# flo-audio/flo

Hardware: AMD Instinct MI355X
Metric: Msamples/s encoded (44.1k stereo, q=high) (higher is better)
Workload: dtype f32

## Files before the change

### flo_amd/csrc/lossy_device.hpp

```cpp
#pragma once
#include <hip/hip_runtime.h>
#include <stdint.h>

#include "pack_rows.h"

namespace flo {


struct LossyDevTables {
    const float4 *pack;
    const float4 *pack_g;
    const float4 *pack_ext;
    const float *ath_db;
    const uint8_t *band;
    const float *band_count;
    const float *s10d;
    const uint32_t *lane_bnd;
    const uint32_t *lane_slot0;
    const uint32_t *band_slot0;
    int max_band_slots;
    uint32_t dirty;
    float smr_thr;
    int q_transparent;
};
// ... 418 lines not shown
    v2f c2r = a4r - a6r, c2i = a4i - a6i;
    v2f c1r = a5r + a7i, c1i = a5i - a7r;
    v2f c3r = a5r - a7i, c3i = a5i + a7r;
    const v2f e1r = c1r + c1i, e1i = c1i - c1r;
    const v2f e3r = c3i - c3r, e3i = c3r + c3i;
    xr[0] = b0r + c0r; xi[0] = b0i + c0i;
    xr[4] = b0r - c0r; xi[4] = b0i - c0i;
    xr[1] = fma2(e1r, s, b1r); xi[1] = fma2(e1i, s, b1i);
    xr[5] = fma2(-e1r, s, b1r); xi[5] = fma2(-e1i, s, b1i);
    xr[2] = b2r + c2i; xi[2] = b2i - c2r;
    xr[6] = b2r - c2i; xi[6] = b2i + c2r;
    xr[3] = fma2(e3r, s, b3r); xi[3] = fma2(-e3i, s, b3i);
    xr[7] = fma2(-e3r, s, b3r); xi[7] = fma2(e3i, s, b3i);
}

__device__ __forceinline__ void cmul_2(v2f &xr, v2f &xi, float wr, float wi) {
    const v2f WR = splat2(wr), WI = splat2(wi);
    v2f r = fma2(xr, WR, -(xi * WI));
    v2f i = fma2(xr, WI, xi * WR);
    xr = r;
    xi = i;
}
__device__ __forceinline__ void cmul_2_pair(v2f &xr, v2f &xi, v2f w) {
    const v2f WR = splat2(w.x);
    v2f r = fma2(xr, WR, -mul2_hi(xi, w));
    v2f i = fma2_a_hi_c(xr, w, xi * WR);
    xr = r;
    xi = i;
}

struct NoShadow { __device__ __forceinline__ void operator()() const {} };
template <typename F = NoShadow>
__device__ __forceinline__ void fft512_2(const int lane, v2f (&zr)[8], v2f (&zi)[8], float4 *x4, const LossyDevTables &T, F &&shadow = F()) {
    dft8_2(zr, zi);
#pragma unroll
    for (int kk = 0; kk < 4; kk++) {
        const float4 w = T.pack[(kRowF1 + kk) * 64 + lane];
        cmul_2(zr[2 * kk + 1], zi[2 * kk + 1], w.x, w.y);
        if (kk < 3) cmul_2_pair(zr[2 * kk + 2], zi[2 * kk + 2], (v2f){w.z, w.w});
    }
    {
        const int nb = lane >> 3, nc = lane & 7;
#pragma unroll
        for (int ka = 0; ka < 8; ka++) x4[(8 * ka + nc) * kXchStride + nb] = make_float4(zr[ka].x, zr[ka].y, zi[ka].x, zi[ka].y);
        wave_sync();
#pragma unroll
        for (int r = 0; r < 8; r++) {
            const float4 v = x4[lane * kXchStride + r];
            zr[r] = (v2f){v.x, v.y};
            zi[r] = (v2f){v.z, v.w};
        }
        shadow();
        wave_sync();
    }
    dft8_2(zr, zi);
#pragma unroll
    for (int kk = 0; kk < 4; kk++) {
        const float4 w = T.pack[(kRowF2 + kk) * 64 + lane];
        cmul_2(zr[2 * kk + 1], zi[2 * kk + 1], w.x, w.y);
        if (kk < 3) cmul_2_pair(zr[2 * kk + 2], zi[2 * kk + 2], (v2f){w.z, w.w});
    }
    {
        const int ka = lane >> 3, nc = lane & 7;
#pragma unroll
        for (int kb = 0; kb < 8; kb++) x4[(ka + 8 * kb) * kXchStride + nc] = make_float4(zr[kb].x, zr[kb].y, zi[kb].x, zi[kb].y);
        wave_sync();
#pragma unroll
        for (int r = 0; r < 8; r++) {
            const float4 v = x4[lane * kXchStride + r];
            zr[r] = (v2f){v.x, v.y};
            zi[r] = (v2f){v.z, v.w};
        }
        wave_sync();
    }
    dft8_2(zr, zi);
}

__device__ __forceinline__ void cmul_2_tw(v2f &xr, v2f &xi, v2f w) {
    const v2f r = fma2_a_lo_nc(xr, w, mul2_hi(xi, w));
    const v2f i = fma2_a_hi_c(xr, w, mul2_lo(xi, w));
    xr = r;
    xi = i;
}
template <typename F = NoShadow>
__device__ __forceinline__ void fft512_2_tw(const int lane, v2f (&zr)[8], v2f (&zi)[8], float4 *x4, const v4f (&f1)[4],
                                            const v4f (&f2)[4], F &&shadow = F()) {
    dft8_2(zr, zi);
#pragma unroll
    for (int kk = 0; kk < 4; kk++) {
        cmul_2_tw(zr[2 * kk + 1], zi[2 * kk + 1], f1[kk].xy);
        if (kk < 3) cmul_2_tw(zr[2 * kk + 2], zi[2 * kk + 2], f1[kk].zw);
    }
    {
        const int nb = lane >> 3, nc = lane & 7;
#pragma unroll
        for (int ka = 0; ka < 8; ka++) x4[(8 * ka + nc) * kXchStride + nb] = make_float4(zr[ka].x, zr[ka].y, zi[ka].x, zi[ka].y);
        wave_sync();
#pragma unroll
        for (int r = 0; r < 8; r++) {
            const float4 v = x4[lane * kXchStride + r];
            zr[r] = (v2f){v.x, v.y};
            zi[r] = (v2f){v.z, v.w};
        }
        shadow();
        wave_sync();
    }
    dft8_2(zr, zi);
#pragma unroll
    for (int kk = 0; kk < 4; kk++) {
        cmul_2_tw(zr[2 * kk + 1], zi[2 * kk + 1], f2[kk].xy);
        if (kk < 3) cmul_2_tw(zr[2 * kk + 2], zi[2 * kk + 2], f2[kk].zw);
    }
    {
        const int ka = lane >> 3, nc = lane & 7;
#pragma unroll
        for (int kb = 0; kb < 8; kb++) x4[(ka + 8 * kb) * kXchStride + nc] = make_float4(zr[kb].x, zr[kb].y, zi[kb].x, zi[kb].y);
        wave_sync();
#pragma unroll
        for (int r = 0; r < 8; r++) {
            const float4 v = x4[lane * kXchStride + r];
            zr[r] = (v2f){v.x, v.y};
            zi[r] = (v2f){v.z, v.w};
        }
        wave_sync();
    }
    dft8_2(zr, zi);
}

__device__ __forceinline__ void load_half_fast_2(const int lane, const float *__restrict__ pcm, long long s0, v2f (&he)[8], v2f (&ho)[8]) {
    const char *base0 = reinterpret_cast<const char *>(pcm + s0 * 2);
    const char *base1 = base0 + 4096;
    const unsigned va = 16u * (unsigned)lane, vb = 16u * (unsigned)(63 - lane);
#pragma unroll
    for (int r = 0; r < 8; r++) {
        const int rr = r & 3;
        const char *pe = (r < 4 ? base1 : base0) + va + 1024 * rr;
        const char *po = (r < 4 ? base0 : base1) + vb + (3080 - 1024 * rr);
        const float2 a = *reinterpret_cast<const float2 *>(pe);
        const float2 b = *reinterpret_cast<const float2 *>(po);
        he[r] = (v2f){a.x, a.y};
        ho[r] = (v2f){b.x, b.y};
    }
}

__device__ __forceinline__ void fold_2(const int lane, const v2f (&ae)[8], const v2f (&ao)[8], const v2f (&be)[8], const v2f (&bo)[8],
                                       v2f (&zr)[8], v2f (&zi)[8], const LossyDevTables &T) {
    float4 t4;
#pragma unroll
    for (int r = 0; r < 8; r++) {
        const float4 ww = T.pack[(kRowWin + r) * 64 + lane];
        const v2f wae = splat2(ww.x), wao = splat2(ww.y), wbe = splat2(ww.z);
        const v2f whi = {ww.z, ww.w};
        if (!(r & 1)) t4 = pack_row(&T.pack[(kRowTw + (r >> 1)) * 64 + lane]);
        const v2f wx = splat2((r & 1) ? t4.z : t4.x);
        const v2f thi = {t4.z, t4.w};
        v2f re, im;
        if (r < 4) {
            re = fma2_na_hi_nc(bo[r], whi, be[r] * wbe);
            im = fma2(ao[r], wao, -(ae[r] * wae));
        } else {
            re = fma2(-ao[r], wao, ae[r] * wae);
            im = fma2_na_hi_nc(bo[r], whi, be[r] * wbe);
        }
        if (r & 1) {
            zr[r] = fma2_na_hi_nc(im, thi, re * wx);
            zi[r] = fma2_a_hi_nc(re, thi, im * wx);
        } else {
            const v2f wy = splat2(t4.y);
            zr[r] = fma2(-im, wy, -(re * wx));
            zi[r] = fma2(re, wy, -(im * wx));
        }
    }
}

__device__ __forceinline__ void post_rotate_transpose_2(const int lane, const v2f (&zr)[8], const v2f (&zi)[8], float2 *c2,
                                                        v2f (&c)[16], const LossyDevTables &T) {
    const int pl = 2 * lane + 2 * (lane >> 3);
    float2 *const w0 = c2 + pl;
    float2 *const w1 = c2 + (1149 - 7 * 144) - pl;
    float4 t4;
#pragma unroll
    for (int r = 0; r < 8; r++) {
        if (!(r & 1)) t4 = pack_row(&T.pack[(kRowTw + (r >> 1)) * 64 + lane]);
        const v2f wx = splat2((r & 1) ? t4.z : t4.x);
        v2f R, I;
        if (r & 1) {
            const v2f thi = {t4.z, t4.w};
            R = fma2_na_hi_nc(zi[r], thi, zr[r] * wx);
            I = fma2(zi[r], wx, -mul2_hi(zr[r], thi));
        } else {
            const v2f wy = splat2(t4.y);
            R = fma2(-zi[r], wy, -(zr[r] * wx));
            I = fma2(zi[r], wx, -(zr[r] * wy));
        }
        w0[144 * r] = make_float2(R.x, R.y);
        w1[144 * (7 - r)] = make_float2(I.x, I.y);
    }
    wave_sync();
    const float4 *p = reinterpret_cast<const float4 *>(&c2[18 * lane]);
#pragma unroll
    for (int q = 0; q < 8; q++) {
        const float4 v = p[q];
        c[2 * q] = (v2f){v.x, v.y};
        c[2 * q + 1] = (v2f){v.z, v.w};
    }
    wave_sync();
}

__device__ __forceinline__ v2f fold_a_part(const int r, const v2f he, const v2f ho, const float4 ww) {
    const v2f wae = splat2(ww.x), wao = splat2(ww.y);
    return r < 4 ? fma2(ho, wao, -(he * wae)) : fma2(-ho, wao, he * wae);
}
__device__ __forceinline__ void fold_carry_init_2(const int lane, v2f (&acar)[8], const LossyDevTables &T) {
#pragma unroll
    for (int r = 0; r < 8; r++) acar[r] = fold_a_part(r, splat2(0.f), splat2(0.f), T.pack[(kRowWin + r) * 64 + lane]);
}
__device__ __forceinline__ void fold_carry_2(const int lane, const v2f (&ne)[8], const v2f (&no)[8], v2f (&acar)[8],
                                             const v4f (&tw)[4], v2f (&zr)[8], v2f (&zi)[8], const LossyDevTables &T) {
#pragma unroll
    for (int r = 0; r < 8; r++) {
        const float4 ww = T.pack[(kRowWin + r) * 64 + lane];
        const v2f wbe = splat2(ww.z);
        const v2f whi = {ww.z, ww.w};
        const v2f t2 = (r & 1) ? tw[r >> 1].zw : tw[r >> 1].xy;
        const v2f bp = fma2_na_hi_nc(no[r], whi, ne[r] * wbe);
        const v2f re = r < 4 ? bp : acar[r], im = r < 4 ? acar[r] : bp;
        zr[r] = fma2_na_hi_nc(im, t2, mul2_lo(re, t2));
        zi[r] = fma2_a_hi_nc(re, t2, mul2_lo(im, t2));
        acar[r] = fold_a_part(r, ne[r], no[r], ww);
    }
}

__device__ __forceinline__ void post_rotate_transpose_2_tw(const int lane, const v2f (&zr)[8], const v2f (&zi)[8], float2 *c2,
                                                           v2f (&c)[16], const v4f (&tw)[4]) {
    const int pl = 2 * lane + 2 * (lane >> 3);
    float2 *const w0 = c2 + pl;
    float2 *const w1 = c2 + (1149 - 7 * 144) - pl;
#pragma unroll
    for (int r = 0; r < 8; r++) {
        const v2f t2 = (r & 1) ? tw[r >> 1].zw : tw[r >> 1].xy;
        const v2f R = fma2_na_hi_nc(zi[r], t2, mul2_lo(zr[r], t2));
        const v2f I = fma2_a_lo_nc(zi[r], t2, mul2_hi(zr[r], t2));
        w0[144 * r] = make_float2(R.x, R.y);
        w1[144 * (7 - r)] = make_float2(I.x, I.y);
    }
    wave_sync();
    const float4 *p = reinterpret_cast<const float4 *>(&c2[18 * lane]);
#pragma unroll
    for (int q = 0; q < 8; q++) {
        const float4 v = p[q];
        c[2 * q] = (v2f){v.x, v.y};
        c[2 * q + 1] = (v2f){v.z, v.w};
    }
    wave_sync();
}

struct LaneConst {
    float rcount;
};

__device__ __forceinline__ void load_lane_const(const int lane, LaneConst &L, const LossyDevTables &T) {
    L.rcount = T.pack[kRowLane * 64 + lane].z;
}

constexpr int kZeroSlot = kSlotCap + 64;

template <int CH>
__device__ __forceinline__ void band_stats(const int lane, const float (&c)[CH][16], float2 (*slots)[kSlotCap + 64 + 1],
                                           const LossyDevTables &T, float (&energy)[CH], float (&bmax)[CH]) {
    float kp[16];
    uint32_t dv[16], so[12];
#pragma unroll
    for (int g = 0; g < 4; g++) {
        const float4 keep = T.pack[(kRowKeep + g) * 64 + lane];
        const float4 dsto = T.pack[(kRowDst + g) * 64 + lane];
        kp[4 * g + 0] = keep.x, kp[4 * g + 1] = keep.y, kp[4 * g + 2] = keep.z, kp[4 * g + 3] = keep.w;
        dv[4 * g + 0] = __float_as_uint(dsto.x), dv[4 * g + 1] = __float_as_uint(dsto.y);
        dv[4 * g + 2] = __float_as_uint(dsto.z), dv[4 * g + 3] = __float_as_uint(dsto.w);
    }
#pragma unroll
    for (int g = 0; g < 3; g++) {
        const float4 lst = T.pack[(kRowLst + g) * 64 + lane];
        so[4 * g + 0] = __float_as_uint(lst.x), so[4 * g + 1] = __float_as_uint(lst.y);
        so[4 * g + 2] = __float_as_uint(lst.z), so[4 * g + 3] = __float_as_uint(lst.w);
    }
    __builtin_amdgcn_sched_barrier(0);
    float acc[CH], mx[CH];
#pragma unroll
    for (int ch = 0; ch < CH; ch++) {
        acc[ch] = 0.f;
        mx[ch] = 0.f;
    }
#pragma unroll
    for (int e = 0; e < 16; e++) {
#pragma unroll
        for (int ch = 0; ch < CH; ch++) {
            acc[ch] = fmaf(c[ch][e], c[ch][e], acc[ch]);
            mx[ch] = max_abs_raw(mx[ch], c[ch][e]);
            *reinterpret_cast<float2 *>(reinterpret_cast<char *>(slots[ch]) + dv[e]) = make_float2(acc[ch], mx[ch]);
            acc[ch] *= kp[e];
            mx[ch] *= kp[e];
        }
    }
    wave_sync();
// ... 164 lines not shown
}

__device__ __forceinline__ float masking_amplitude(float s, float smr_thr) {
    const float thr_db = s - 10.0f;
    return __builtin_amdgcn_exp2f((smr_thr + thr_db) * 0.16609640474436813f);
}

__device__ __forceinline__ uint32_t sf_word(float sf) {
    if (sf > 1e-10f) {
        float v = __builtin_amdgcn_logf(sf) * 256.0f + 32768.0f;
        v = __builtin_amdgcn_fmed3f(v, 0.0f, 65535.0f);
        return (uint32_t)v;
    }
    return 0u;
}

__device__ __forceinline__ float round_away(float x) {
    float t = truncf(x);
    float d = x - t;
    return t + truncf(d + d);
}

template <int CH, bool EXACT>
__device__ __forceinline__ void quantise(const int lane, const float (&c)[CH][16], const WaveLds<CH> &lds, const LaneConst &L,
                                         const LossyDevTables &T, int (&q)[CH][16]) {
    float al[16];
    uint32_t bo[16];
#pragma unroll
    for (int g = 0; g < 4; g++) {
        const float4 al4 = T.pack[(kRowAth + g) * 64 + lane];
        const float4 bo4 = T.pack[(kRowBo + g) * 64 + lane];
        al[4 * g + 0] = al4.x, al[4 * g + 1] = al4.y, al[4 * g + 2] = al4.z, al[4 * g + 3] = al4.w;
        bo[4 * g + 0] = __float_as_uint(bo4.x), bo[4 * g + 1] = __float_as_uint(bo4.y);
        bo[4 * g + 2] = __float_as_uint(bo4.z), bo[4 * g + 3] = __float_as_uint(bo4.w);
    }
    __builtin_amdgcn_sched_barrier(0);
    float2 bv[CH][16];
#pragma unroll
    for (int e = 0; e < 16; e++)
#pragma unroll
        for (int ch = 0; ch < CH; ch++)
            bv[ch][e] = *reinterpret_cast<const float2 *>(reinterpret_cast<const char *>(lds.bandv[ch]) + bo[e]);
    __builtin_amdgcn_sched_barrier(0);
#pragma unroll
    for (int e = 0; e < 16; e++) {
#pragma unroll
        for (int ch = 0; ch < CH; ch++) {
            const float x = c[ch][e];
            const float ax = fabsf(x);
            const float thr = max_raw(bv[ch][e].x, al[e]);
            const float xs = x * bv[ch][e].y;
            const float half = __uint_as_float((__float_as_uint(xs) & 0x80000000u) | 0x3EFFFFFFu);
            const int v = cvt_rz(xs + half);
            if (EXACT) {
                bool keep = ax > thr;
                const bool near = fabsf(ax - thr) <= 1e-5f * thr || (T.q_transparent && !(ax > 1e-10f));
                if (near) {
                    float signal_db = ax > 1e-10f ? 20.0f * log10f(ax) : -100.0f;
                    float sdb = *reinterpret_cast<const float *>(reinterpret_cast<const char *>(lds.band_s[ch]) + (bo[e] >> 1));
                    float t = fmaxf(sdb, T.ath_db[16 * lane + e]) - 10.0f;
                    keep = (signal_db - t) > T.smr_thr;
                }
                q[ch][e] = keep ? v : 0;
            } else {
                const int mask = __float_as_int(thr - ax) >> 31;
                q[ch][e] = v & mask;
            }
        }
    }
}

constexpr int kSlots = kSlotCap + 64 + 1;
struct StereoLds {
    union {
        float4 xch4[kXch4];
        float2 coef2[kCoef2];
        struct {
            float4 slot[kSlots];
            float4 ts[32];
        } a;
    } u;
};

template <uint32_t DIRTY = 0xFFFFu, bool SO_PRE = false, bool MASKS = false>
__device__ __forceinline__ void band_stats_2(const int lane, const v2f (&c)[16], float4 *slot, const LossyDevTables &T,
                                             float &energy1, float &bmax1, const uint32_t *so_pre = nullptr,
                                             const unsigned long long *close = nullptr, const uint32_t slot_first = 0) {
    static_assert(!MASKS || SO_PRE, "the masked form takes its addresses from band_stats_2_prepare");
    typedef float v4f __attribute__((ext_vector_type(4)));
    typedef __attribute__((address_space(3))) v4f lds_v4f;
    const uint32_t s0 = (uint32_t)__builtin_amdgcn_readfirstlane((int)(uint32_t)(uintptr_t)slot);
    if (!SO_PRE) {
        typedef __attribute__((address_space(3))) float lds_f32;
        float z = 0.f;
        asm volatile("" : "+v"(z));
        *reinterpret_cast<lds_f32 *>((uintptr_t)(s0 + 16u * (uint32_t)kZeroSlot + 4u * ((uint32_t)lane & 3u))) = z;
    }
    uint32_t so[12];
#pragma unroll
    for (int g = 0; g < 3; g++) {
        if (SO_PRE) {
            so[4 * g + 0] = so_pre[4 * g + 0], so[4 * g + 1] = so_pre[4 * g + 1], so[4 * g + 2] = so_pre[4 * g + 2], so[4 * g + 3] = so_pre[4 * g + 3];
        } else {
            const float4 lst = T.pack[(kRowLst + g) * 64 + lane];
            so[4 * g + 0] = s0 + 2u * __float_as_uint(lst.x), so[4 * g + 1] = s0 + 2u * __float_as_uint(lst.y);
            so[4 * g + 2] = s0 + 2u * __float_as_uint(lst.z), so[4 * g + 3] = s0 + 2u * __float_as_uint(lst.w);
        }
    }
    const uint32_t dirty = DIRTY;
    v4f am = {0.f, 0.f, 0.f, 0.f};
    uint32_t sa = slot_first;
#pragma unroll
    for (int g = 0; g < 4; g++) {
        const float4 keep = MASKS ? make_float4(0.f, 0.f, 0.f, 0.f) : pack_row(&T.pack[(kRowKeep + g) * 64 + lane]);
        const float4 dsto = MASKS ? make_float4(0.f, 0.f, 0.f, 0.f) : pack_row(&T.pack[(kRowDst + g) * 64 + lane]);
        const float kp[4] = {keep.x, keep.y, keep.z, keep.w};
        const uint32_t dv[4] = {__float_as_uint(dsto.x), __float_as_uint(dsto.y), __float_as_uint(dsto.z), __float_as_uint(dsto.w)};
#pragma unroll
        for (int k = 0; k < 4; k++) {
            const int e = 4 * g + k;
            am.xy = fma2(c[e], c[e], am.xy);
            const bool prev_open = e > 0 && !((dirty >> (e - 1)) & 1u), this_open = e < 15 && !((dirty >> e) & 1u);
            if (prev_open) {
                am.z = max3_abs_raw(am.z, c[e - 1].x, c[e].x);
                am.w = max3_abs_raw(am.w, c[e - 1].y, c[e].y);
            } else if (!this_open) {
                am.z = max_abs_raw(am.z, c[e].x);
                am.w = max_abs_raw(am.w, c[e].y);
            }
            if (MASKS && ((dirty >> e) & 1u)) {
                if (e < 15) {
                    v2f lo = am.xy, hi = am.zw;
                    unsigned long long saved;
                    asm volatile("s_and_saveexec_b64 %[sv], %[m]\n\t"
                                 "ds_write2_b64 %[a], %[lo], %[hi] offset1:1\n\t"
                                 "v_add_u32 %[a], 16, %[a]\n\t"
                                 "v_pk_mul_f32 %[lo], %[lo], 0 op_sel_hi:[1,0]\n\t"
                                 "v_pk_mul_f32 %[hi], %[hi], 0 op_sel_hi:[1,0]\n\t"
                                 "s_mov_b64 exec, %[sv]"
                                 : [a] "+v"(sa), [lo] "+v"(lo), [hi] "+v"(hi), [sv] "=&s"(saved)
                                 : [m] "s"(close[e])
                                 : "memory");
                    am.xy = lo, am.zw = hi;
                } else {
                    *reinterpret_cast<lds_v4f *>((uintptr_t)sa) = am;
                }
            } else if ((dirty >> e) & 1u) {
                *reinterpret_cast<lds_v4f *>((uintptr_t)(s0 + 2u * dv[k])) = am;
                if (e < 15) {
                    am.xy = am.xy * splat2(kp[k]);
                    am.zw = am.zw * splat2(kp[k]);
                }
            }
        }
    }
    wave_sync();
    v2f energy = splat2(0.f), bmax = splat2(0.f);
#pragma unroll
    for (int g = 0; g < 3; g++) {
        v4f v[4];
#pragma unroll
        for (int u = 0; u < 4; u++) v[u] = *reinterpret_cast<const lds_v4f *>((uintptr_t)so[4 * g + u]);
#pragma unroll
        for (int u = 0; u < 4; u++) energy = energy + (v2f){v[u].x, v[u].y};
#pragma unroll
        for (int u = 0; u < 4; u += 2) {
            bmax.x = max3_raw(bmax.x, v[u].z, v[u + 1].z);
            bmax.y = max3_raw(bmax.y, v[u].w, v[u + 1].w);
        }
    }
    const int groups = (T.max_band_slots + 7) >> 3;
    for (int g = 3; g < groups; g++) {
        const float4 lst = g < 6 ? T.pack_g[(kRowLstCold + g - 3) * 64 + lane] : T.pack_ext[(g - 6) * 64 + lane];
        const uint32_t sx[4] = {__float_as_uint(lst.x), __float_as_uint(lst.y), __float_as_uint(lst.z), __float_as_uint(lst.w)};
        v4f w[4];
#pragma unroll
        for (int u = 0; u < 4; u++) w[u] = *reinterpret_cast<const lds_v4f *>((uintptr_t)(s0 + 2u * sx[u]));
#pragma unroll
        for (int u = 0; u < 4; u++) {
            energy = energy + (v2f){w[u].x, w[u].y};
            bmax.x = max_raw(bmax.x, w[u].z);
            bmax.y = max_raw(bmax.y, w[u].w);
        }
    }
    {
        const auto e2 = __builtin_amdgcn_permlane32_swap(__float_as_int(energy.x), __float_as_int(energy.y), false, false);
        const auto m2 = __builtin_amdgcn_permlane32_swap(__float_as_int(bmax.x), __float_as_int(bmax.y), false, false);
        energy1 = __int_as_float(e2[0]) + __int_as_float(e2[1]);
        bmax1 = max_raw(__int_as_float(m2[0]), __int_as_float(m2[1]));
    }
    wave_sync();
}

__device__ __forceinline__ void band_stats_2_prepare(const int lane, float4 *slot, const float4 *pack, uint32_t (&so)[12],
                                                     uint32_t &slot_first) {
    const uint32_t s0 = (uint32_t)(uintptr_t)slot;
    slot_first = s0 + 16u * reinterpret_cast<const uint32_t *>(pack + kRowLane * 64 + lane)[1];
    if (lane < 4) reinterpret_cast<float *>(slot + kZeroSlot)[lane] = 0.f;
#pragma unroll
    for (int g = 0; g < 3; g++) {
        const float4 lst = pack[(kRowLst + g) * 64 + lane];
        so[4 * g + 0] = s0 + 2u * __float_as_uint(lst.x), so[4 * g + 1] = s0 + 2u * __float_as_uint(lst.y);
        so[4 * g + 2] = s0 + 2u * __float_as_uint(lst.z), so[4 * g + 3] = s0 + 2u * __float_as_uint(lst.w);
    }
}
template <uint32_t DIRTY>
__device__ __forceinline__ void band_stats_2_masks(const StatMasks *masks, unsigned long long (&close)[16]) {
#pragma unroll
    for (int e = 0; e < 16; e++) {
        const bool used = e < 15 && ((DIRTY >> e) & 1u);
        close[e] = used ? masks->close[e] : 0ull;
        if (used) asm volatile("" : "+s"(close[e]));
    }
}

struct QuantRows {
    float4 bo4[4];
};
__device__ __forceinline__ void quant_rows_load(const int lane, const LossyDevTables &T, QuantRows &R) {
#pragma unroll
    for (int g = 0; g < 4; g++) {
        R.bo4[g] = T.pack[(kRowBo + g) * 64 + lane];
    }
}
__device__ __forceinline__ void quantise_2(const int lane, const v2f (&c)[16], const float4 *ts, const LossyDevTables &T,
                                           const QuantRows &R, uint32_t (&xs)[2][8]) {
    typedef float v4f __attribute__((ext_vector_type(4)));
    typedef __attribute__((address_space(3))) v4f lds_f4;
    const uint32_t ts0 = (uint32_t)__builtin_amdgcn_readfirstlane((int)(uint32_t)(uintptr_t)ts);
    const uint32_t sgn_mask = 0x7FFFFFFFu;
    uint32_t phalf = 0x3EFFFFFFu;
    asm volatile("" : "+v"(phalf));
#pragma unroll
    for (int g = 0; g < 4; g++) {
        const float4 al4 = T.pack[(kRowAth + g) * 64 + lane];
        const float4 bo4 = R.bo4[g];
        const float al[4] = {al4.x, al4.y, al4.z, al4.w};
        const uint32_t bo[4] = {__float_as_uint(bo4.x), __float_as_uint(bo4.y), __float_as_uint(bo4.z), __float_as_uint(bo4.w)};
        v4f tb[4];
#pragma unroll
        for (int k = 0; k < 4; k++) tb[k] = *reinterpret_cast<const lds_f4 *>((uintptr_t)(ts0 + 2u * bo[k]));
        int v[2][4];
// ... 548 lines not shown
```

### flo_amd/csrc/lossy_kernels.hip

```cpp
#include <assert.h>
#include <stdlib.h>

#include <mutex>
#include <set>
#include <type_traits>
#include <utility>

#include "chain2q_roles.hpp"
#include "crc_device.hpp"
#include "lossy_device.hpp"
#include "lossy_kernels.hpp"
#include "../../include/flo_synth.h"

#ifndef FLO_SKIP
#define FLO_SKIP 0
#endif
#define FLO_KEEP(x) asm volatile("" ::"v"(x))
#ifdef FLO_STAMPS
#define STAMP(i)                                                                                  \
    do {                                                                                          \
        __builtin_amdgcn_sched_barrier(0);                                                        \
        unsigned long long t_;                                                                    \
        asm volatile("s_memtime %0\n\ts_waitcnt lgkmcnt(0)" : "=s"(t_)::"memory");              \
        __builtin_amdgcn_sched_barrier(0);                                                        \
// ... 616 lines not shown
    float ath_floor = masks->band_ath_floor[lane & 31];
    asm volatile("" : "+v"(ath_floor));
    v4f tw[4];
    v4f f1[4], f2[4];
    if (!COEFFS) {
#pragma unroll
        for (int k = 0; k < 4; k++) tw[k] = pack_row_v(&T.pack[(kRowTw + k) * 64 + lane]);
#pragma unroll
        for (int k = 0; k < 4; k++) f1[k] = pack_row_v(&T.pack[(kRowF1 + k) * 64 + lane]);
#pragma unroll
        for (int k = 0; k < 4; k++) f2[k] = pack_row_v(&T.pack[(kRowF2 + k) * 64 + lane]);
    }
    for (;;) {
        wait_counter(&cs.clip_seq, ++seq);
        const unsigned clip = (unsigned)__builtin_amdgcn_readfirstlane((int)cs.clip_cur);
        if (clip >= (unsigned)A.n_clips) return;
        const unsigned hops = A.clip_hops[clip];
        const unsigned long long frame0 = A.clip_frame0[clip];
        const float *pcm = A.pcm + A.clip_off[clip];

        float prev = 0.f;
        v2f ne[8], no[8], acar[8];
        if (!COEFFS) {
            fold_carry_init_2(lane_id_opaque(), acar, T);
            load_half_fast_2(lane_id_opaque(), pcm, 0, ne, no);
        }
        STAMPS_BEGIN();
        v2f zr[8], zi[8];
        if (!COEFFS) fold_carry_2(lane_id_opaque(), ne, no, acar, tw, zr, zi, T);
        float pend_e = 0.f, pend_m = 0.f;
        auto mask_publish = [&](const int ln, const uint32_t gp, const unsigned hp, const float energy1, const float bmax1,
                                const float rcount, const float4 sd0, const float4 sd1) __attribute__((always_inline)) {
            const int bnd = ln & 31, up = ln >> 5;
#if (FLO_SKIP & 16) == 0
            const float bm = bmax1;
            const float sfv1 = bm > 1e-10f ? __fdiv_rn(30000.0f, bm) : 1.0f;
            const uint32_t sfw1 = sf_word(sfv1);
            const float a = spread_threshold_2r(ln, energy1, rcount, sd0, sd1, T);
            const float sl = max_raw(a, prev * 0.7f);
            prev = sl;
            const float tl1 = masking_amplitude(sl, T.smr_thr);
#else
            const float bm = bmax1, tl1 = energy1 * 1e-3f + rcount + sd0.x + sd1.y, sfv1 = bm * 100.f + 1.f;
            const uint32_t sfw1 = __float_as_uint(tl1) >> 16;
#endif
            const unsigned long long al = __ballot(bnd < 25 && bm > tl1 && bm > ath_floor);
            if (bnd < 25) {
                typedef __attribute__((address_space(3))) float lds_f32;
                const uint32_t ts_s = (uint32_t)__builtin_amdgcn_readfirstlane((int)(uint32_t)(uintptr_t)cs.ts[gp & 1u]);
                lds_f32 *tp = reinterpret_cast<lds_f32 *>((uintptr_t)(ts_s + 16u * (uint32_t)bnd + 4u * (uint32_t)up));
                tp[0] = tl1;
                tp[2] = sfv1;
                cs.sfwh[gp & 1u][up][bnd] = (uint16_t)sfw1;
            }
            if (ln == 0) {
                cs.alive[gp & 1u][0] = (uint32_t)al;
                cs.alive[gp & 1u][1] = (uint32_t)(al >> 32);
            }
            if (DBG && A.dbg_sfw && bnd < 25) A.dbg_sfw[((frame0 + hp) * 2 + up) * 25 + bnd] = (unsigned short)sfw1;
            set_counter(&cs.ts_ready, gp + 1);
        };
        auto frame_body = [&](const unsigned h) __attribute__((always_inline)) {
            const int ln = lane_id_opaque();
            const uint32_t g = fbase + h;
            FLO_MARK("frame_begin");
            const uint32_t consumed_early = peek_counter(&cs.consumed);
            const float4 sd0 = T.pack[kRowS10 * 64], sd1 = T.pack[kRowS10 * 64 + 1];
            const float rcount = reinterpret_cast<const float *>(T.pack + kRowS10 * 64)[64 + ln];
            v2f c[16];
            if (COEFFS) {
#pragma unroll
                for (int q = 0; q < 4; q++) {
                    const float4 v0 = reinterpret_cast<const float4 *>(A.in_coeffs + ((frame0 + h) * 2 + 0) * 1024 + 16 * ln)[q];
                    const float4 v1 = reinterpret_cast<const float4 *>(A.in_coeffs + ((frame0 + h) * 2 + 1) * 1024 + 16 * ln)[q];
                    c[4 * q] = (v2f){v0.x, v1.x}; c[4 * q + 1] = (v2f){v0.y, v1.y};
                    c[4 * q + 2] = (v2f){v0.z, v1.z}; c[4 * q + 3] = (v2f){v0.w, v1.w};
                }
                if ((uint32_t)__builtin_amdgcn_readfirstlane((int)consumed_early) < g) wait_counter(&cs.consumed, g);
                float4 *p = reinterpret_cast<float4 *>(&cs.u.coef2[18 * ln]);
#pragma unroll
                for (int q = 0; q < 8; q++) p[q] = make_float4(c[2 * q].x, c[2 * q].y, c[2 * q + 1].x, c[2 * q + 1].y);
                wave_sync();
            } else {
                STAMP(1);
                if ((uint32_t)__builtin_amdgcn_readfirstlane((int)consumed_early) < g) wait_counter(&cs.consumed, g);
                STAMP(7);
#if (FLO_SKIP & 8) == 0
                fft512_2_tw(ln, zr, zi, cs.u.xch4, f1, f2, [&]() __attribute__((always_inline)) {
                    if (h > 0) mask_publish(ln, g - 1u, h - 1u, pend_e, pend_m, rcount, sd0, sd1);
                });
#else
                if (h > 0) mask_publish(ln, g - 1u, h - 1u, pend_e, pend_m, rcount, sd0, sd1);
#endif
                FLO_MARK("fft_done");
                STAMP(2);
                load_half_fast_2(ln, pcm, (long long)(h + 1) * 1024, ne, no);
                FLO_MARK("prefetch_done");
#if (FLO_SKIP & 4) == 0
                post_rotate_transpose_2_tw(ln, zr, zi, cs.u.coef2, c, tw);
#else
#pragma unroll
                for (int e = 0; e < 8; e++) { c[2 * e] = zr[e]; c[2 * e + 1] = zi[e]; }
#endif
                FLO_MARK("postrot_done");
                STAMP(3);
                if (DBG && A.dbg_coeffs) {
#pragma unroll
                    for (int ch = 0; ch < 2; ch++) {
                        float *d = A.dbg_coeffs + ((frame0 + h) * 2 + ch) * 1024 + 16 * ln;
#pragma unroll
                        for (int e = 0; e < 16; e++) d[e] = ch ? c[e].y : c[e].x;
                    }
                }
            }
            set_counter(&cs.coef_ready, g + 1);
            float energy1, bmax1;
#if (FLO_SKIP & 1) == 0
            band_stats_2<DIRTY, true, true>(ln, c, cs.slot, T, energy1, bmax1, so_pre, close, slot_first);
#else
            energy1 = c[0].x + c[5].y;
            bmax1 = c[1].x + c[7].y;
#endif
            FLO_MARK("bandstats_done");
            STAMP(4);
            if (COEFFS) {
                mask_publish(ln, g, h, energy1, bmax1, rcount, sd0, sd1);
            } else {
                pend_e = energy1, pend_m = bmax1;
#if (FLO_SKIP & 128) == 0
                fold_carry_2(ln, ne, no, acar, tw, zr, zi, T);
#else
#pragma unroll
                for (int r = 0; r < 8; r++) { zr[r] = acar[r] + ne[r]; zi[r] = acar[r] - no[r]; }
#endif
            }
            FLO_MARK("frame_end");
            STAMP(5);
        };
        for (unsigned h = 0; h < hops; h++) frame_body(h);
        if (!COEFFS && hops) {
            const int ln = lane_id_opaque();
            const float4 sd0 = T.pack[kRowS10 * 64], sd1 = T.pack[kRowS10 * 64 + 1];
            mask_publish(ln, fbase + hops - 1u, hops - 1u, pend_e, pend_m, reinterpret_cast<const float *>(T.pack + kRowS10 * 64)[64 + ln], sd0, sd1);
        }
        STAMPS_RECORD(0);
        fbase += hops;
    }
}

template <int CH, int STEP, bool EXACT>
__global__ __launch_bounds__(64) void lossy_frame_kernel(LossyArgs A) {
    constexpr int PASS = STEP & ~kStreamStep;
    constexpr bool STREAM = (STEP & kStreamStep) != 0;
    __shared__ WaveLds<CH> lds;
    __shared__ __attribute__((aligned(16))) uint8_t stage[kFrameCap + 64 + 256];
    const int lane = lane_id();
    const unsigned long long gframe = blockIdx.x;
    if (gframe >= A.total_frames) return;
    int lo = 0, hi = A.n_clips - 1;
    while (lo < hi) {
        int mid = (lo + hi + 1) >> 1;
        if (A.clip_frame0[mid] <= gframe) lo = mid; else hi = mid - 1;
    }
    const unsigned clip = (unsigned)lo;
    const unsigned h = (unsigned)(gframe - A.clip_frame0[clip]);
    const float *pcm = A.pcm + A.clip_off[clip];
    const long long n_sf = (long long)A.clip_nsf[clip];

    LaneConst L;
    load_lane_const(lane, L, A.T);
    if (lane < CH) lds.slots[lane][kZeroSlot] = make_float2(0.f, 0.f);
    float c[CH][16];
    if (A.in_coeffs) {
        load_coeffs<CH>(lane, c, A, gframe, 0);
    } else {
        float ae[CH][8], ao[CH][8], be[CH][8], bo[CH][8];
        load_half<CH>(lane, pcm, n_sf, A.nch, 0, (long long)(h + STREAM) * 1024 - 1024, ae, ao);
        load_half<CH>(lane, pcm, n_sf, A.nch, 0, (long long)(h + STREAM) * 1024, be, bo);
        mdct_frame<CH>(lane, ae, ao, be, bo, lds, A.T, c);
    }
    FrameState<CH> st;
    int q[CH][16];
    uint32_t sfw[CH];
    SparsePlan P[CH];
    if (PASS == 1) {
#pragma unroll
        for (int ch = 0; ch < CH; ch++) st.prev[ch] = 0.f;
        analyse_frame<CH, true, EXACT>(lane, c, lds, L, A, A.T, 0, st, gframe, q, sfw, P);
        if (lane < 25) {
#pragma unroll
            for (int ch = 0; ch < CH; ch++) mark_inf_level(A, clip, (unsigned)ch, (unsigned)lane, h, A.a_t[(gframe * A.nch + ch) * 32 + lane]);
        }
        return;
    }
    store_coeffs_dbg<CH>(lane, c, A, gframe, 0);
#pragma unroll
    for (int ch = 0; ch < CH; ch++) st.prev[ch] = lane < 25 ? A.s_prev[(gframe * A.nch + ch) * 32 + lane] : 0.f;
    analyse_frame<CH, false, EXACT>(lane, c, lds, L, A, A.T, 0, st, gframe, q, sfw, P);
    uint32_t tot[2];
    tot[0] = P[0].total;
    tot[1] = P[CH - 1].total;
    const uint32_t flen = emit_frame<CH>(lane, stage, CH, 0, tot, sfw, P, q);
    wave_sync();
    if (lane == 0) A.frame_size[gframe] = flen;
    const uint32_t n16 = (flen + 15) >> 4;
    const uint4 *src = reinterpret_cast<const uint4 *>(stage);
    uint4 *dst = reinterpret_cast<uint4 *>(A.slots + gframe * (unsigned long long)A.slot_bytes);
    for (uint32_t i = lane; i < n16; i += 64) dst[i] = src[i];
}

constexpr int kScanBlock = 64;
struct QuantOnlyLds {
    float4 ts[32];
// ... 911 lines not shown
```

Baseline: 734,200.

## Hide LDS and table-load latency by interleaving work into wait shadows

Several latency-hiding rearrangements in the encode frame body. The buffer-free counter wait moves to just before the first FFT exchange write, so the first radix stage runs before it. The second twiddle multiply is interleaved with the LDS stores. The window table rows in fold_carry are software-pipelined one row ahead, with the first row issued inside the band-stats gather shadow. Band-stats gathers for the masked path are issued in batches separated by sched_barriers. A diagnostic script for counting short LDS wait shadows is also added. The sched_barriers pin instruction order, which could limit the compiler's own scheduling or raise register pressure.

```diff
diff --git a/diag/wait_shadow.py b/diag/wait_shadow.py
--- /dev/null
+++ b/diag/wait_shadow.py
@@ -0,0 +1,85 @@
+#!/usr/bin/env python3
+import re
+import sys
+
+
+def main():
+    argv = sys.argv[1:]
+    below = None
+    if "--below" in argv:
+        k = argv.index("--below")
+        below = int(argv[k + 1])
+        del argv[k:k + 2]
+    path = argv[0]
+    want = argv[1] if len(argv) > 1 else "lossy_chain2q_kernelILb0ELj48574ELb0EE"
+    lines = open(path).read().split("\n")
+    start = next(i for i, l in enumerate(lines) if l.startswith("_Z") and want in l and ":" in l.split(";")[0])
+    end = next(i for i in range(start, len(lines)) if ".size" in lines[i] and want in lines[i])
+    marks = [(i, re.match(r"; MARK (\w+)", lines[i].strip()).group(1)) for i in range(start, end) if lines[i].strip().startswith("; MARK ")]
+    first = {n: min(i for i, m in marks if m == n) for n in {m for _, m in marks}}
+    is_label = lambda j: re.match(r"\.LBB\d+_\d+:", lines[j])
+    label_at = lambda i: max(j for j in range(start, i + 1) if is_label(j))
+    header = label_at(first["frame_begin"])
+    if first["frame_end"] < first["frame_begin"]:
+        loop_start = label_at(marks[0][0])
+        leave = next(lines[j] for j in range(header - 1, loop_start, -1) if lines[j].strip().startswith("s_cbranch"))
+        post_start = next(j for j in range(start, end) if lines[j].startswith(leave.split()[1] + ":"))
+        latch = lines[loop_start].split(":")[0]
+        back = next((j for j in range(header, post_start) if re.match(r"s_c?branch\S*\s+" + re.escape(latch) + r"\b", lines[j].strip())), post_start - 1)
+        order = list(range(header, back + 1)) + list(range(loop_start, header))
+    else:
+        order = list(range(header, first["frame_end"] + 1))
+    def depth_of(j):
+        k = j
+        while True:
+            m = re.search(r"(?:Loop Header:|in Loop: Header=\S+) Depth=(\d+)", lines[k])
+            if m:
+                return int(m.group(1))
+            k += 1
+            if not lines[k].startswith(" ") or ";" not in lines[k] or lines[k].split(";")[0].strip():
+                return 0
+    frame_depth = depth_of(header)
+
+    rows, outstanding, cur, inner, smem = [], [], "frame_end", False, 0
+    for i in order:
+        s = lines[i].strip()
+        if is_label(i) or s.startswith("; %bb."):
+            inner = depth_of(i) > frame_depth
+            continue
+        m = re.match(r"; MARK (\w+)", s)
+        if m:
+            cur = m.group(1)
+            continue
+        if inner or not s or s.startswith((";", ".", "//")):
+            continue
+        op = s.split()[0]
+        if op.startswith("ds_"):
+            outstanding.append([i, s.split(";")[0].strip(), 0])
+        elif op.startswith(("s_load", "s_buffer_load")):
+            smem += 1
+        elif op.startswith(("v_", "global_", "buffer_", "flat_", "scratch_")):
+            for o in outstanding:
+                o[2] += 1
+        elif op == "s_waitcnt":
+            m = re.search(r"lgkmcnt\((\d+)\)", s)
+            if not m:
+                continue
+            n = int(m.group(1))
+            if len(outstanding) > n:
+                awaited = outstanding[len(outstanding) - n - 1]
+                rows.append((cur, i + 1, n, awaited[1], awaited[2], len(outstanding) - n))
+                outstanding = outstanding[len(outstanding) - n:]
+    names = {"frame_begin": "fft + masking pass", "fft_done": "prefetch", "prefetch_done": "post-rotation", "postrot_done": "band statistics",
+             "bandstats_done": "next fold (a)", "frame_end": "next fold (b), loop"}
+    shown = [r for r in rows if below is None or r[4] < below]
+    print(f"{'behind marker':15s} {'phase':20s} {'line':>6s} {'lgkmcnt':>7s} {'shadow':>6s} {'done':>4s}  awaited instruction")
+    for cur, ln, n, txt, sh, done in shown:
+        print(f"{cur:15s} {names.get(cur, cur):20s} {ln:6d} {n:7d} {sh:6d} {done:4d}  {' '.join(txt.split())}")
+    short = sum(1 for r in rows if r[4] < 8)
+    print(f"{len(rows)} LDS waits in the frame body, {short} with fewer than 8 vector instructions in their shadow"
+          + (f"; {smem} SMEM loads between the markers (they share lgkmcnt)" if smem else ""))
+    return 1 if below is not None and shown else 0
+
+
+if __name__ == "__main__":
+    sys.exit(main())
diff --git a/flo_amd/csrc/lossy_device.hpp b/flo_amd/csrc/lossy_device.hpp
--- a/flo_amd/csrc/lossy_device.hpp
+++ b/flo_amd/csrc/lossy_device.hpp
@@ -524,15 +524,16 @@
     xr = r;
     xi = i;
 }
-template <typename F = NoShadow>
+template <typename F = NoShadow, typename G = NoShadow>
 __device__ __forceinline__ void fft512_2_tw(const int lane, v2f (&zr)[8], v2f (&zi)[8], float4 *x4, const v4f (&f1)[4],
-                                            const v4f (&f2)[4], F &&shadow = F()) {
+                                            const v4f (&f2)[4], F &&shadow = F(), G &&before_x4 = G()) {
     dft8_2(zr, zi);
 #pragma unroll
     for (int kk = 0; kk < 4; kk++) {
         cmul_2_tw(zr[2 * kk + 1], zi[2 * kk + 1], f1[kk].xy);
         if (kk < 3) cmul_2_tw(zr[2 * kk + 2], zi[2 * kk + 2], f1[kk].zw);
     }
+    before_x4();
     {
         const int nb = lane >> 3, nc = lane & 7;
 #pragma unroll
@@ -548,15 +549,21 @@
         wave_sync();
     }
     dft8_2(zr, zi);
-#pragma unroll
-    for (int kk = 0; kk < 4; kk++) {
-        cmul_2_tw(zr[2 * kk + 1], zi[2 * kk + 1], f2[kk].xy);
-        if (kk < 3) cmul_2_tw(zr[2 * kk + 2], zi[2 * kk + 2], f2[kk].zw);
-    }
     {
         const int ka = lane >> 3, nc = lane & 7;
-#pragma unroll
-        for (int kb = 0; kb < 8; kb++) x4[(ka + 8 * kb) * kXchStride + nc] = make_float4(zr[kb].x, zr[kb].y, zi[kb].x, zi[kb].y);
+        auto put = [&](const int kb) __attribute__((always_inline)) {
+            x4[(ka + 8 * kb) * kXchStride + nc] = make_float4(zr[kb].x, zr[kb].y, zi[kb].x, zi[kb].y);
+        };
+        put(0);
+#pragma unroll
+        for (int kk = 0; kk < 4; kk++) {
+            cmul_2_tw(zr[2 * kk + 1], zi[2 * kk + 1], f2[kk].xy);
+            put(2 * kk + 1);
+            if (kk < 3) {
+                cmul_2_tw(zr[2 * kk + 2], zi[2 * kk + 2], f2[kk].zw);
+                put(2 * kk + 2);
+            }
+        }
         wave_sync();
 #pragma unroll
         for (int r = 0; r < 8; r++) {
@@ -658,10 +665,15 @@
     for (int r = 0; r < 8; r++) acar[r] = fold_a_part(r, splat2(0.f), splat2(0.f), T.pack[(kRowWin + r) * 64 + lane]);
 }
 __device__ __forceinline__ void fold_carry_2(const int lane, const v2f (&ne)[8], const v2f (&no)[8], v2f (&acar)[8],
-                                             const v4f (&tw)[4], v2f (&zr)[8], v2f (&zi)[8], const LossyDevTables &T) {
+                                             const v4f (&tw)[4], v2f (&zr)[8], v2f (&zi)[8], const LossyDevTables &T,
+                                             const float4 *win0 = nullptr) {
+    float4 wrow[8];
+    wrow[0] = win0 ? *win0 : T.pack[kRowWin * 64 + lane];
 #pragma unroll
     for (int r = 0; r < 8; r++) {
-        const float4 ww = T.pack[(kRowWin + r) * 64 + lane];
+        if (r + 1 < 8) wrow[r + 1] = T.pack[(kRowWin + r + 1) * 64 + lane];
+        __builtin_amdgcn_sched_barrier(0);
+        const float4 ww = wrow[r];
         const v2f wbe = splat2(ww.z);
         const v2f whi = {ww.z, ww.w};
         const v2f t2 = (r & 1) ? tw[r >> 1].zw : tw[r >> 1].xy;
@@ -992,10 +1004,11 @@
     } u;
 };
 
-template <uint32_t DIRTY = 0xFFFFu, bool SO_PRE = false, bool MASKS = false>
+template <uint32_t DIRTY = 0xFFFFu, bool SO_PRE = false, bool MASKS = false, typename R = NoShadow>
 __device__ __forceinline__ void band_stats_2(const int lane, const v2f (&c)[16], float4 *slot, const LossyDevTables &T,
                                              float &energy1, float &bmax1, const uint32_t *so_pre = nullptr,
-                                             const unsigned long long *close = nullptr, const uint32_t slot_first = 0) {
+                                             const unsigned long long *close = nullptr, const uint32_t slot_first = 0,
+                                             R &&behind_gathers = R()) {
     static_assert(!MASKS || SO_PRE, "the masked form takes its addresses from band_stats_2_prepare");
     typedef float v4f __attribute__((ext_vector_type(4)));
     typedef __attribute__((address_space(3))) v4f lds_v4f;
@@ -1066,8 +1079,33 @@
     }
     wave_sync();
     v2f energy = splat2(0.f), bmax = splat2(0.f);
-#pragma unroll
-    for (int g = 0; g < 3; g++) {
+    if (MASKS) {
+        v4f v[8];
+        auto take4 = [&](const int b) __attribute__((always_inline)) {
+#pragma unroll
+            for (int u = 0; u < 4; u++) energy = energy + (v2f){v[b + u].x, v[b + u].y};
+#pragma unroll
+            for (int u = 0; u < 4; u += 2) {
+                bmax.x = max3_raw(bmax.x, v[b + u].z, v[b + u + 1].z);
+                bmax.y = max3_raw(bmax.y, v[b + u].w, v[b + u + 1].w);
+            }
+        };
+#pragma unroll
+        for (int u = 0; u < 8; u++) v[u] = *reinterpret_cast<const lds_v4f *>((uintptr_t)so[u]);
+        __builtin_amdgcn_sched_barrier(0);
+        take4(0);
+        __builtin_amdgcn_sched_barrier(0);
+#pragma unroll
+        for (int u = 0; u < 4; u++) v[u] = *reinterpret_cast<const lds_v4f *>((uintptr_t)so[8 + u]);
+        __builtin_amdgcn_sched_barrier(0);
+        take4(4);
+        __builtin_amdgcn_sched_barrier(0);
+        behind_gathers();
+        __builtin_amdgcn_sched_barrier(0);
+        take4(0);
+    }
+#pragma unroll
+    for (int g = MASKS ? 3 : 0; g < 3; g++) {
         v4f v[4];
 #pragma unroll
         for (int u = 0; u < 4; u++) v[u] = *reinterpret_cast<const lds_v4f *>((uintptr_t)so[4 * g + u]);
diff --git a/flo_amd/csrc/lossy_kernels.hip b/flo_amd/csrc/lossy_kernels.hip
--- a/flo_amd/csrc/lossy_kernels.hip
+++ b/flo_amd/csrc/lossy_kernels.hip
@@ -722,14 +722,17 @@
                 for (int q = 0; q < 8; q++) p[q] = make_float4(c[2 * q].x, c[2 * q].y, c[2 * q + 1].x, c[2 * q + 1].y);
                 wave_sync();
             } else {
-                STAMP(1);
-                if ((uint32_t)__builtin_amdgcn_readfirstlane((int)consumed_early) < g) wait_counter(&cs.consumed, g);
-                STAMP(7);
+                auto buffer_free = [&]() __attribute__((always_inline)) {
+                    STAMP(1);
+                    if ((uint32_t)__builtin_amdgcn_readfirstlane((int)consumed_early) < g) wait_counter(&cs.consumed, g);
+                    STAMP(7);
+                };
 #if (FLO_SKIP & 8) == 0
                 fft512_2_tw(ln, zr, zi, cs.u.xch4, f1, f2, [&]() __attribute__((always_inline)) {
                     if (h > 0) mask_publish(ln, g - 1u, h - 1u, pend_e, pend_m, rcount, sd0, sd1);
-                });
+                }, buffer_free);
 #else
+                buffer_free();
                 if (h > 0) mask_publish(ln, g - 1u, h - 1u, pend_e, pend_m, rcount, sd0, sd1);
 #endif
                 FLO_MARK("fft_done");
@@ -755,9 +758,13 @@
             }
             set_counter(&cs.coef_ready, g + 1);
             float energy1, bmax1;
+            float4 win0;
 #if (FLO_SKIP & 1) == 0
-            band_stats_2<DIRTY, true, true>(ln, c, cs.slot, T, energy1, bmax1, so_pre, close, slot_first);
+            band_stats_2<DIRTY, true, true>(ln, c, cs.slot, T, energy1, bmax1, so_pre, close, slot_first, [&]() __attribute__((always_inline)) {
+                if (!COEFFS) win0 = T.pack[kRowWin * 64 + ln];
+            });
 #else
+            if (!COEFFS) win0 = T.pack[kRowWin * 64 + ln];
             energy1 = c[0].x + c[5].y;
             bmax1 = c[1].x + c[7].y;
 #endif
@@ -768,7 +775,7 @@
             } else {
                 pend_e = energy1, pend_m = bmax1;
 #if (FLO_SKIP & 128) == 0
-                fold_carry_2(ln, ne, no, acar, tw, zr, zi, T);
+                fold_carry_2(ln, ne, no, acar, tw, zr, zi, T, &win0);
 #else
 #pragma unroll
                 for (int r = 0; r < 8; r++) { zr[r] = acar[r] + ne[r]; zi[r] = acar[r] - no[r]; }
```

After: 739,100 (median of 6 runs). Within noise of the previous version (+0.7%).
